# zju3dv/disprcnn

Measured on AMD Instinct MI355X. Metric: ROI cost-volumes/sec (112x112x48), higher is better.
Workload: dtype f32 (every convolution of the regressor, the three 32->1 heads included: split-f16 -- each fp32 value carried as hi + lo fp16, 3 f16-MFMA products per fp32 product, f32 accumulate; fp32-class error, tests/test_hip_s16.py.  Head gather and soft-argmin: f32 VALU); 1 GPU; Config A: per ROI pair, features [32,28,28]x2 -> concat cost volume [64,12,28,28] (folded into the first 3D layer's loads, never written) -> 3D stacked-hourglass regressor -> trilinear x4 + softmax + soft-argmin -> disparity [112,112]; maxdisp=48, mindisp=0, parallelism=roi-shard x1 (no collective), weights=closed-form synthetic (disprcnn_amd.utils.synth), BN stats calibrated fixture

## Files before the change

### disprcnn_amd/csrc/convs16.hip

```cpp
#include <hip/hip_runtime.h>
#include <stdint.h>

#include <type_traits>

#include "../../include/disprcnn_hip.h"
#include "s16_cvrows.h"
#include "s16_ovf.h"
#include "s16_tilemap.h"

typedef float f32x4 __attribute__((ext_vector_type(4)));
typedef float f32x16 __attribute__((ext_vector_type(16)));
typedef unsigned u32x4 __attribute__((ext_vector_type(4)));
typedef unsigned u32x2 __attribute__((ext_vector_type(2)));
typedef _Float16 f16x8 __attribute__((ext_vector_type(8)));
typedef _Float16 f16x4 __attribute__((ext_vector_type(4)));

#define GLOBAL_PTR(p) ((const __attribute__((address_space(1))) void*)(p))
#define LDS_PTR(p) ((__attribute__((address_space(3))) void*)(p))
#define S16_WAITCNT(vm, lgkm) (((vm) & 15) | (7 << 4) | ((lgkm) << 8) | (((vm) >> 4) << 14))

namespace {

constexpr int PV = 128;
constexpr int CPB = PV * 16;
constexpr int RING = 3;

template <int KW, bool CV, int RT = 1, int WT = 28, bool RES = false, bool Y32 = false, bool HEAD = false>
__global__ __launch_bounds__(256) __attribute__((amdgpu_waves_per_eu(1, 1))) void convs16_kernel(const drc_s16conv_params p) {
    static_assert(!HEAD || (KW == 2 && !CV && RT == 1 && !RES && !Y32), "the fused cout-1 head is a form of the 32 -> 32 full-resolution layer");
    static_assert(!CV || (KW == 4 && RT == 1 && WT == 28 && !RES && !Y32), "the cost-volume form: 64 virtual input channels, full-resolution rows, RS16 output");
    extern __shared__ __attribute__((aligned(16))) char lds[];
    if constexpr (CV) {
        s16cv::s16_cvrows_run<1>(p, lds);
        return;
    }
    constexpr int TX = WT;
    constexpr int SX = WT + 2;
    constexpr int RPW = 4 / KW;
    constexpr int CBI = KW / 2;
    constexpr int SROWS = RPW * RT + 2;
    static_assert(RT * WT <= 32, "tile shape");
    constexpr int SLAB = CBI * 8 * CPB;
    constexpr int NL = CBI * 8 * (PV / 64) / 4;
    constexpr int OWN = 16 / KW;
    constexpr int XW = 4096;
    constexpr int NR = RES ? 2 : 0;
    constexpr int NS = 2;
    static_assert(!(Y32 && (KW != 2 || RES)), "the blocked fp32 output exists for the 32-channel layers without residual");
    static_assert(RT == 1 ? SROWS * SX + 4 <= PV : (SROWS + 1) * SX + 4 <= PV, "slab plane too small (incl. the rows / columns the idle lanes over-read)");
    char* ring = lds;
    char* xchg = lds + RING * SLAB;
    char* pbuf = xchg + 2 * 4 * XW;

    const int wave = __builtin_amdgcn_readfirstlane(threadIdx.x >> 6);
    const int lane = threadIdx.x & 63;
    const int n_ = lane & 31, g = lane >> 5;
    const S16TileLane tln = s16_tile_lane<RT, WT>(n_, !(p.lo4 & 0x100));
    const int rl = tln.rl, xl = tln.xl;
    const int r = wave / KW, k = wave % KW;
    const int n_ct = p.cout / 32;
    const int ct = (int)((blockIdx.x >> 3) % n_ct);

    const int D = p.D, H = p.H, W = p.W;
    const int Wp = W + 2, Hp = H + 2;
    const long rowB = (long)Wp * 128;
    const long planeB = (long)Hp * rowB;
    const long xcbB = (long)(D + 2) * planeB;
    const long xnB = (long)CBI * xcbB;
    const int cbo = p.cout / 32;
    const long ynB = (long)cbo * xcbB;
    const long b_rowB = (long)Wp * 64, b_planeB = (long)Hp * b_rowB, b_cbB = (long)(D + 2) * b_planeB, b_nB = (long)(p.cout / 16) * b_cbB;

    f16x8 wh[27], wl[27];
    {
        const char* wb = (const char*)p.w + ((long)(ct * KW + k) * 54) * 1024 + lane * 16;
#pragma unroll
        for (int t = 0; t < 27; ++t) {
            wh[t] = *(const f16x8*)(wb + (t * 2) * 1024);
            wl[t] = *(const f16x8*)(wb + (t * 2 + 1) * 1024);
        }
    }
    float sc[OWN], sh[OWN];
#pragma unroll
    for (int e = 0; e < OWN; ++e) {
        const int reg = k * OWN + e;
        const int co = ct * 32 + (reg & 3) + 8 * (reg >> 2) + 4 * g;
        sc[e] = p.scale[co];
        sh[e] = p.shift[co];
    }
    f16x8 w1h = {}, w1l = {};
    if constexpr (HEAD) {
        const char* wb = (const char*)p.w1 + (long)k * 2048 + lane * 16;
        w1h = *(const f16x8*)wb;
        w1l = *(const f16x8*)(wb + 1024);
    }
    int srcrow[2], srcx[2];
    bool srcok[2];
#pragma unroll
    for (int h = 0; h < 2; ++h) {
        const int v = h * 64 + lane;
        srcok[h] = v < SROWS * SX;
        const int rr = srcok[h] ? v / SX : 0;
        srcrow[h] = rr;
        srcx[h] = srcok[h] ? v - rr * SX : 0;
    }
    const unsigned bfrag = (unsigned)(((k >> 1) * 8 + (k & 1) * 2 + g) * CPB + ((r * RT + rl) * SX + xl) * 16);
    const __attribute__((address_space(3))) char* ringl = (const __attribute__((address_space(3))) char*)ring;
    typedef const __attribute__((address_space(3))) f16x8 lds_frag;

    const int n_xt = (W + TX - 1) / TX, n_yt = (H + RPW * RT - 1) / (RPW * RT);
    const int Dw = (D + 2) / 3 * 3;
    const unsigned xcd = blockIdx.x & 7, qx = (blockIdx.x >> 3) / n_ct, per_xcd = (gridDim.x >> 3) / n_ct;
    const unsigned cols_unit = (unsigned)n_yt * n_xt;

    struct Col { unsigned n; int y0, x0; bool valid; };
    auto col_of = [&](unsigned it) __attribute__((always_inline)) {
        const unsigned j = it * per_xcd + qx;
        const unsigned nl = j / cols_unit;
        const unsigned rem = j - nl * cols_unit;
        const int yb = (int)(rem / n_xt), xt = (int)(rem - (unsigned)yb * n_xt);
        Col c;
        c.n = nl * 8 + xcd;
        c.valid = c.n < (unsigned)p.N;
        c.y0 = yb * RPW * RT;
        c.x0 = xt * TX;
        return c;
    };
    struct Src { const char* a; unsigned v0, v1; };
    auto src_of = [&](const Col& c) __attribute__((always_inline)) {
        Src q;
        q.a = (const char*)p.x + (long)c.n * xnB;
        q.v0 = (unsigned)((long)(c.y0 + srcrow[0]) * rowB + (long)(c.x0 + srcx[0]) * 16);
        q.v1 = (unsigned)((long)(c.y0 + srcrow[1]) * rowB + (long)(c.x0 + srcx[1]) * 16);
        return q;
    };
    auto stage = [&](const Src& q, int pl, int slot) __attribute__((always_inline)) {
        char* dst = ring + slot * SLAB;
        const __amdgpu_buffer_rsrc_t ra = __builtin_amdgcn_make_buffer_rsrc((void*)q.a, 0, 0x7FFFFF00, 0x00020000);
        const unsigned va[2] = {q.v0, q.v1};
#pragma unroll
        for (int i = 0; i < NL; ++i) {
            const int id = wave * NL + i;
            const int cb = id >> 4, c = (id >> 1) & 7, h = id & 1;
            const int so = (int)((long)cb * xcbB + (long)(pl + 1) * planeB + (long)c * (Wp * 16));
            __builtin_amdgcn_raw_ptr_buffer_load_lds(ra, LDS_PTR(dst + (cb * 8 + c) * CPB + h * 1024), 16, va[h], so, 0, 0);
        }
    };
    const long hs_planeB = (long)H * W * 48, hs_nB = (long)D * hs_planeB;
    struct Ctx { char* y16b; char* y32b; const char* resb; char* hsb; unsigned o16, o32, ohs; bool ok; };
    auto ctx_of = [&](const Col& c) __attribute__((always_inline)) {
        Ctx q;
        q.hsb = HEAD ? (char*)p.head + (long)c.n * hs_nB : (char*)p.w;
        q.ohs = (unsigned)(((long)(c.y0 + r * RT + rl) * W + (c.x0 + xl)) * 48 + g * 32);
        q.y16b = p.y16 ? (char*)p.y16 + (long)c.n * ynB : (char*)p.w;
        q.y32b = p.y32 ? (char*)p.y32 + (long)c.n * b_nB : (char*)p.w;
        q.resb = p.res ? (const char*)p.res + (long)c.n * ynB : (const char*)p.w;
        const int yl = c.y0 + r * RT + rl;
        q.ok = tln.ok && yl < H && c.x0 + xl < W;
        if constexpr (KW == 2) {
            q.o16 = (unsigned)((long)ct * xcbB + planeB + (long)(yl + 1) * rowB + (long)(k * 2 + g) * (Wp * 16) + (long)(c.x0 + xl + 1) * 16);
            q.o32 = (unsigned)((long)(2 * ct + k) * b_cbB + b_planeB + (long)(yl + 1) * b_rowB + (long)(c.x0 + xl + 1) * 64 + g * 16);
        } else {
            q.o16 = (unsigned)((long)ct * xcbB + planeB + (long)(yl + 1) * rowB + (long)((k >> 1) * 2 + g) * (Wp * 16) + (long)(c.x0 + xl + 1) * 16 + (k & 1) * 8);
            q.o32 = (unsigned)((long)(2 * ct + (k >> 1)) * b_cbB + b_planeB + (long)(yl + 1) * b_rowB + (long)(c.x0 + xl + 1) * 64 + (k & 1) * 32 + g * 16);
        }
        return q;
    };
    const unsigned lo_off = (unsigned)(4 * Wp * 16);
    const float relu_lo = p.relu ? 0.f : -65504.f;
    const unsigned n16 = p.y16 ? 0x7FFFFF00u : 0u, n32 = p.y32 ? 0x7FFFFF00u : 0u, nres = p.res ? 0x7FFFFF00u : 0u;

    Col ccur = col_of(0);
    if (!ccur.valid) return;
    S16Ovf og;
#pragma unroll
    for (int e = 0; e < OWN; ++e) { og.see_raw(sc[e], 3.0e38f); og.see_raw(sh[e], 3.0e38f); }
    Src s_cur = src_of(ccur), s_next = s_cur;
    Ctx cx_cur = ctx_of(ccur), cx_prev = cx_cur;
    cx_prev.ok = false;

    f32x16 acc[3];
    u32x4 resv[3][2];
#pragma unroll
    for (int a_ = 0; a_ < 3; ++a_)
#pragma unroll
        for (int e = 0; e < 16; ++e) acc[a_][e] = 0.f;
#pragma unroll
    for (int a_ = 0; a_ < 3; ++a_) resv[a_][0] = resv[a_][1] = (u32x4){0u, 0u, 0u, 0u};
    f32x16 pkeep = {};
    float SC[5] = {0.f, 0.f, 0.f, 0.f, 0.f}, SB[5] = {0.f, 0.f, 0.f, 0.f, 0.f};
    stage(s_cur, 0, 0);
    stage(s_cur, 1 < D ? 1 : D, 1);
    __builtin_amdgcn_s_waitcnt(S16_WAITCNT(NL, 15));
    unsigned gs = 0;

    auto step = [&](int t, auto JT, auto KT) __attribute__((always_inline)) {
        constexpr int J = decltype(JT)::value;
        constexpr int KIND = decltype(KT)::value;
        constexpr bool COMPUTE = KIND != 3;
        constexpr int A0 = (J + 1) % 3, A1 = J, A2 = (J + 2) % 3;
        asm volatile("" ::: "memory");
        __builtin_amdgcn_s_waitcnt(S16_WAITCNT(NL + NS + NR, 0));
        __builtin_amdgcn_s_barrier();
        asm volatile("" ::: "memory");
        const bool fcur = t >= 2, pcur = t >= 1;
        const int qf = fcur ? t - 2 : Dw - 2 + t, qp = pcur ? t - 1 : Dw - 1;
        const __amdgpu_buffer_rsrc_t resr = __builtin_amdgcn_make_buffer_rsrc((void*)(pcur ? cx_cur.resb : cx_prev.resb), 0, nres, 0x00020000);
        const unsigned p_o16 = pcur ? cx_cur.o16 : cx_prev.o16;
        const bool p_ok = (pcur ? cx_cur.ok : cx_prev.ok) && qp >= 0 && qp < D;
        if constexpr (RES) {
            const unsigned po = p_ok ? (unsigned)((long)qp * planeB) : 0x80000000u;
            if constexpr (KW == 2) {
                resv[J][0] = __builtin_amdgcn_raw_buffer_load_b128(resr, p_o16 + po, 0, 0);
                resv[J][1] = __builtin_amdgcn_raw_buffer_load_b128(resr, p_o16 + lo_off + po, 0, 0);
            } else {
                const u32x2 a_ = __builtin_amdgcn_raw_buffer_load_b64(resr, p_o16 + po, 0, 0);
                const u32x2 b_ = __builtin_amdgcn_raw_buffer_load_b64(resr, p_o16 + lo_off + po, 0, 0);
                resv[J][0] = (u32x4){a_.x, a_.y, 0u, 0u};
                resv[J][1] = (u32x4){b_.x, b_.y, 0u, 0u};
            }
        }
        {
            const int tp = t + 2;
            const bool nxt = tp >= Dw;
            Src q;
            q.a = nxt ? s_next.a : s_cur.a;
            q.v0 = nxt ? s_next.v0 : s_cur.v0;
            q.v1 = nxt ? s_next.v1 : s_cur.v1;
            int pl = nxt ? tp - Dw : tp;
            pl = pl < D ? pl : D;
            stage(q, pl, (J + 2) % 3);
        }
        const __amdgpu_buffer_rsrc_t y16r = __builtin_amdgcn_make_buffer_rsrc(fcur ? cx_cur.y16b : cx_prev.y16b, 0, n16, 0x00020000);
        const __amdgpu_buffer_rsrc_t y32r = __builtin_amdgcn_make_buffer_rsrc(fcur ? cx_cur.y32b : cx_prev.y32b, 0, n32, 0x00020000);
        const unsigned f_o16 = fcur ? cx_cur.o16 : cx_prev.o16, f_o32 = fcur ? cx_cur.o32 : cx_prev.o32;
        const bool f_ok = (fcur ? cx_cur.ok : cx_prev.ok) && qf >= 0 && qf < D;
        f32x4 part[4];
        {
            const char* xb = xchg + ((gs - 1) & 1) * (4 * XW) + (r * KW) * XW + lane * 16;
            if constexpr (KW == 2) {
                part[0] = *(const f32x4*)(xb + (k * 2) * 1024);
                part[1] = *(const f32x4*)(xb + XW + (k * 2) * 1024);
                part[2] = *(const f32x4*)(xb + (k * 2 + 1) * 1024);
                part[3] = *(const f32x4*)(xb + XW + (k * 2 + 1) * 1024);
            } else {
#pragma unroll
                for (int q = 0; q < 4; ++q) part[q] = *(const f32x4*)(xb + q * XW + k * 1024);
            }
        }
        f32x4 pin[4];
        if constexpr (HEAD) {
            const char* pb = pbuf + ((gs - 1) & 1) * (2 * XW) + r * XW + lane * 16;
#pragma unroll
            for (int q = 0; q < 4; ++q) pin[q] = *(const f32x4*)(pb + q * 1024);
        }
        if constexpr (RES) {
            __builtin_amdgcn_s_waitcnt(S16_WAITCNT(2 * NL + NS + NR, 15));
            __builtin_amdgcn_sched_barrier(0);
        }
        float v[OWN];
        _Float16 vh[OWN], vl[OWN];
        const unsigned long long og_keep = S16Ovf::lanes(f_ok);
        auto fin = [&](int e) __attribute__((always_inline)) {
            float s_;
            if constexpr (KW == 2) s_ = part[(e >> 2) * 2][e & 3] + part[(e >> 2) * 2 + 1][e & 3];
            else s_ = (part[0][e] + part[1][e]) + (part[2][e] + part[3][e]);
            float x_ = s_ * sc[e] + sh[e];
            if constexpr (RES) {
                const _Float16 rh = __builtin_bit_cast(f16x8, resv[(J + 2) % 3][0])[e], rl_ = __builtin_bit_cast(f16x8, resv[(J + 2) % 3][1])[e];
                x_ += (float)rh + (float)rl_;
            }
            x_ = __builtin_amdgcn_fmed3f(x_, relu_lo, 65504.f);
            og.see(x_, og_keep);
            v[e] = x_;
            vh[e] = (_Float16)x_;
            vl[e] = (_Float16)(x_ - (float)vh[e]);
        };
        auto stores = [&]() __attribute__((always_inline)) {
            if constexpr (Y32) {
                const unsigned po32 = f_ok ? (unsigned)((long)qf * b_planeB) : 0x80000000u;
                __builtin_amdgcn_raw_buffer_store_b128(__builtin_bit_cast(u32x4, (f32x4){v[0], v[1], v[2], v[3]}), y32r, f_o32 + po32, 0, 0);
                __builtin_amdgcn_raw_buffer_store_b128(__builtin_bit_cast(u32x4, (f32x4){v[4], v[5], v[6], v[7]}), y32r, f_o32 + 32 + po32, 0, 0);
            } else {
                const unsigned po = f_ok ? (unsigned)((long)qf * planeB) : 0x80000000u;
                if constexpr (KW == 2) {
                    f16x8 hi, lo;
#pragma unroll
                    for (int e = 0; e < 8; ++e) { hi[e] = vh[e]; lo[e] = vl[e]; }
                    __builtin_amdgcn_raw_buffer_store_b128(__builtin_bit_cast(u32x4, hi), y16r, f_o16 + po, 0, 0);
                    __builtin_amdgcn_raw_buffer_store_b128(__builtin_bit_cast(u32x4, lo), y16r, f_o16 + lo_off + po, 0, 0);
                } else {
                    f16x4 hi, lo;
#pragma unroll
                    for (int e = 0; e < 4; ++e) { hi[e] = vh[e]; lo[e] = vl[e]; }
                    __builtin_amdgcn_raw_buffer_store_b64(__builtin_bit_cast(u32x2, hi), y16r, f_o16 + po, 0, 0);
                    __builtin_amdgcn_raw_buffer_store_b64(__builtin_bit_cast(u32x2, lo), y16r, f_o16 + lo_off + po, 0, 0);
                }
            }
        };
        auto publish = [&]() __attribute__((always_inline)) {
            const f32x16 a = acc[A2];
            char* xb = xchg + (gs & 1) * (4 * XW) + wave * XW + lane * 16;
#pragma unroll
            for (int q = 0; q < 4; ++q) *(f32x4*)(xb + q * 1024) = (f32x4){a[q * 4], a[q * 4 + 1], a[q * 4 + 2], a[q * 4 + 3]};
#pragma unroll
            for (int e = 0; e < 16; ++e) acc[A2][e] = 0.f;
        };
        float o_[5];
        f32x16 z_ = {};
        f16x8 bh_ = {}, bl_ = {};
        auto head_update = [&](int jj) __attribute__((always_inline)) {
            if constexpr (HEAD) {
                const bool first = t == 3;
                const float p0 = pkeep[3 * jj] + pin[(3 * jj) >> 2][(3 * jj) & 3];
                const float p1 = pkeep[3 * jj + 1] + pin[(3 * jj + 1) >> 2][(3 * jj + 1) & 3];
                const float p2 = pkeep[3 * jj + 2] + pin[(3 * jj + 2) >> 2][(3 * jj + 2) & 3];
                o_[jj] = SC[jj] + (first ? 0.f : p2);
                SC[jj] = (first ? 0.f : SB[jj]) + p1;
                SB[jj] = p0;
            }
        };
        auto head_store = [&]() __attribute__((always_inline)) {
            if constexpr (HEAD) {
                const bool scur = t >= 4;
                const int ps = scur ? t - 4 : Dw - 4 + t;
                const bool ok_ = k == 0 && (scur ? cx_cur.ok : cx_prev.ok) && ps >= 0 && ps < D;
                const __amdgpu_buffer_rsrc_t hsr = __builtin_amdgcn_make_buffer_rsrc(scur ? cx_cur.hsb : cx_prev.hsb, 0, 0x7FFFFF00, 0x00020000);
                const unsigned oh_ = scur ? cx_cur.ohs : cx_prev.ohs;
                const unsigned po = ok_ ? (unsigned)((long)ps * hs_planeB) : 0x80000000u;
                __builtin_amdgcn_raw_buffer_store_b128(__builtin_bit_cast(u32x4, (f32x4){o_[0], o_[1], o_[2], o_[3]}), hsr, oh_ + po, 0, 0);
                __builtin_amdgcn_raw_buffer_store_b32(__builtin_bit_cast(unsigned, o_[4]), hsr, oh_ + 16 + (g ? 0x80000000u : po), 0, 0);
            }
        };
        auto head_mfma = [&](int i) __attribute__((always_inline)) {
            if constexpr (HEAD) {
                if (i == 0) {
#pragma unroll
                    for (int e = 0; e < 8; ++e) { bh_[e] = vh[e]; bl_[e] = vl[e]; }
                    z_ = __builtin_amdgcn_mfma_f32_32x32x16_f16(w1h, bh_, z_, 0, 0, 0);
                } else if (i == 1) {
                    z_ = __builtin_amdgcn_mfma_f32_32x32x16_f16(w1h, bl_, z_, 0, 0, 0);
                } else {
                    z_ = __builtin_amdgcn_mfma_f32_32x32x16_f16(w1l, bh_, z_, 0, 0, 0);
                    pkeep = z_;
                    if (k == 1) {
                        char* pb = pbuf + (gs & 1) * (2 * XW) + r * XW + lane * 16;
#pragma unroll
                        for (int q = 0; q < 4; ++q) *(f32x4*)(pb + q * 1024) = (f32x4){z_[q * 4], z_[q * 4 + 1], z_[q * 4 + 2], z_[q * 4 + 3]};
                    }
                }
            }
        };
        if constexpr (COMPUTE) {
            constexpr bool K0 = KIND != 2, K2 = KIND != 1;
            const __attribute__((address_space(3))) char* sb = ringl + J * SLAB + bfrag;
            f16x8 bh[2], bl[2];
            bh[0] = *(lds_frag*)(sb);
            bl[0] = *(lds_frag*)(sb + 4 * CPB);
#pragma unroll
            for (int q = 0; q < 9; ++q) {
                const int kh = q / 3, kw = q - kh * 3;
                if (q + 1 < 9) {
                    const int kh1 = (q + 1) / 3, kw1 = (q + 1) - kh1 * 3;
                    bh[(q + 1) & 1] = *(lds_frag*)(sb + (kh1 * SX + kw1) * 16);
                    bl[(q + 1) & 1] = *(lds_frag*)(sb + 4 * CPB + (kh1 * SX + kw1) * 16);
                }
                const f16x8 h_ = bh[q & 1], l_ = bl[q & 1];
                const int t0 = kh * 3 + kw, t1 = 9 + t0, t2 = 18 + t0;
                if (q == OWN && !HEAD) stores();
                if (q < 8) {
                    if (K0) acc[A0] = __builtin_amdgcn_mfma_f32_32x32x16_f16(wh[t0], h_, acc[A0], 0, 0, 0);
                    acc[A1] = __builtin_amdgcn_mfma_f32_32x32x16_f16(wh[t1], h_, acc[A1], 0, 0, 0);
                    if (K2) acc[A2] = __builtin_amdgcn_mfma_f32_32x32x16_f16(wh[t2], h_, acc[A2], 0, 0, 0);
                    if (K0) acc[A0] = __builtin_amdgcn_mfma_f32_32x32x16_f16(wh[t0], l_, acc[A0], 0, 0, 0);
                    acc[A1] = __builtin_amdgcn_mfma_f32_32x32x16_f16(wh[t1], l_, acc[A1], 0, 0, 0);
                    if (K2) acc[A2] = __builtin_amdgcn_mfma_f32_32x32x16_f16(wh[t2], l_, acc[A2], 0, 0, 0);
                    if (K0) acc[A0] = __builtin_amdgcn_mfma_f32_32x32x16_f16(wl[t0], h_, acc[A0], 0, 0, 0);
                    acc[A1] = __builtin_amdgcn_mfma_f32_32x32x16_f16(wl[t1], h_, acc[A1], 0, 0, 0);
                    if (K2) acc[A2] = __builtin_amdgcn_mfma_f32_32x32x16_f16(wl[t2], h_, acc[A2], 0, 0, 0);
                    if (q < OWN) fin(q);
                    if (q < 5) head_update(q);
                    if (q == 5) head_store();
                    __builtin_amdgcn_sched_barrier(0);
                } else {
                    if (K2) acc[A2] = __builtin_amdgcn_mfma_f32_32x32x16_f16(wh[t2], h_, acc[A2], 0, 0, 0);
                    if (K0) acc[A0] = __builtin_amdgcn_mfma_f32_32x32x16_f16(wh[t0], h_, acc[A0], 0, 0, 0);
                    head_mfma(0);
                    if (K2) acc[A2] = __builtin_amdgcn_mfma_f32_32x32x16_f16(wh[t2], l_, acc[A2], 0, 0, 0);
                    acc[A1] = __builtin_amdgcn_mfma_f32_32x32x16_f16(wh[t1], h_, acc[A1], 0, 0, 0);
                    if (K2) acc[A2] = __builtin_amdgcn_mfma_f32_32x32x16_f16(wl[t2], h_, acc[A2], 0, 0, 0);
                    __builtin_amdgcn_sched_barrier(0);
                    head_mfma(1);
                    if (K0) acc[A0] = __builtin_amdgcn_mfma_f32_32x32x16_f16(wh[t0], l_, acc[A0], 0, 0, 0);
                    acc[A1] = __builtin_amdgcn_mfma_f32_32x32x16_f16(wh[t1], l_, acc[A1], 0, 0, 0);
                    if (K0) acc[A0] = __builtin_amdgcn_mfma_f32_32x32x16_f16(wl[t0], h_, acc[A0], 0, 0, 0);
                    acc[A1] = __builtin_amdgcn_mfma_f32_32x32x16_f16(wl[t1], h_, acc[A1], 0, 0, 0);
                    publish();
                    head_mfma(2);
                }
            }
        } else {
#pragma unroll
            for (int e = 0; e < OWN; ++e) fin(e);
            if constexpr (HEAD) {
#pragma unroll
                for (int jj = 0; jj < 5; ++jj) head_update(jj);
                head_store();
                head_mfma(0); head_mfma(1); head_mfma(2);
            } else {
                stores();
            }
            publish();
        }
        ++gs;
    };
    using I0 = std::integral_constant<int, 0>;
    using I1 = std::integral_constant<int, 1>;
    using I2 = std::integral_constant<int, 2>;
    using I3 = std::integral_constant<int, 3>;
#pragma unroll 1
    for (unsigned it = 0;; ++it) {
        const Col cnext = col_of(it + 1);
        s_next = cnext.valid ? src_of(cnext) : s_cur;
        step(0, I0{}, I1{});
        step(1, I1{}, I0{});
        if (Dw == 3) {
            step(2, I2{}, I2{});
        } else {
            step(2, I2{}, I0{});
#pragma unroll 1
            for (int t0 = 3; t0 + 3 < Dw; t0 += 3) {
                step(t0, I0{}, I0{});
                step(t0 + 1, I1{}, I0{});
                step(t0 + 2, I2{}, I0{});
            }
            step(Dw - 3, I0{}, I0{});
            step(Dw - 2, I1{}, I0{});
            step(Dw - 1, I2{}, I2{});
        }
        if (!cnext.valid) break;
        cx_prev = cx_cur;
        cx_cur = ctx_of(cnext);
        s_cur = s_next;
    }
    step(Dw, I0{}, I3{});
    step(Dw + 1, I1{}, I3{});
    if constexpr (HEAD) {
        step(Dw + 2, I2{}, I3{});
        const bool ok_ = k == 0 && cx_cur.ok;
        const __amdgpu_buffer_rsrc_t hsr = __builtin_amdgcn_make_buffer_rsrc(cx_cur.hsb, 0, 0x7FFFFF00, 0x00020000);
        const unsigned po = ok_ ? (unsigned)((long)(D - 1) * hs_planeB) : 0x80000000u;
        __builtin_amdgcn_raw_buffer_store_b128(__builtin_bit_cast(u32x4, (f32x4){SC[0], SC[1], SC[2], SC[3]}), hsr, cx_cur.ohs + po, 0, 0);
        __builtin_amdgcn_raw_buffer_store_b32(__builtin_bit_cast(unsigned, SC[4]), hsr, cx_cur.ohs + 16 + (g ? 0x80000000u : po), 0, 0);
    }
    og.flush(p.ovf);
}

template <int KW, bool CV, int RT, int WT, bool RES, bool Y32, bool HEAD = false>
int launch2(const drc_s16conv_params& p, hipStream_t stream) {
    constexpr int CBI = KW / 2;
    constexpr int SLAB = CBI * 8 * CPB;
    constexpr int XW = 4096;
    constexpr size_t lds = CV ? (size_t)s16cv::LDS_BYTES : RING * SLAB + 2 * 4 * XW + (HEAD ? 2 * 2 * XW : 0);
    static_assert(lds <= 160 * 1024, "LDS");
    static bool attr_done = false;
    if (!attr_done) {
        (void)hipFuncSetAttribute((const void*)convs16_kernel<KW, CV, RT, WT, RES, Y32, HEAD>, hipFuncAttributeMaxDynamicSharedMemorySize, 160 * 1024);
        attr_done = true;
    }
    constexpr int rows = (4 / KW) * RT;
    const long columns = (long)p.N * ((p.H + rows - 1) / rows) * ((p.W + WT - 1) / WT);
    const int n_ct = p.cout / 32;
    long blocks = 256;
    while (blocks > 8 * n_ct && blocks / (2 * n_ct) >= columns) blocks /= 2;
    if constexpr (CV) blocks = s16cv::s16_cvrows_blocks<1>(p);
    hipLaunchKernelGGL((convs16_kernel<KW, CV, RT, WT, RES, Y32, HEAD>), dim3((unsigned)blocks), dim3(256), lds, stream, p);
    return (int)hipGetLastError();
}

template <int KW, bool CV, int RT = 1, int WT = 28>
int launch(const drc_s16conv_params& p, hipStream_t stream) {
    if (p.head) {
        if constexpr (KW == 2 && !CV && RT == 1) return launch2<KW, CV, RT, WT, false, false, true>(p, stream);
        else return -4;
    }
    if (p.y32) {
        if constexpr (KW == 2 && !CV && RT == 1) return launch2<KW, CV, RT, WT, false, true>(p, stream);
        else return -4;
    }
    if constexpr (CV) return launch2<KW, CV, RT, WT, false, false>(p, stream);
    else return p.res ? launch2<KW, CV, RT, WT, true, false>(p, stream) : launch2<KW, CV, RT, WT, false, false>(p, stream);
}

}

extern "C" int drc_conv3d_k3_s16_supported(int cin, int cout, int D, int H, int W) {
    if (cin != 32 && cin != 64) return 0;
    if (cout != 32 && cout != 64) return 0;
    return D > 0 && H > 0 && W > 0;
}

extern "C" int drc_conv3d_k3_s16_fwd(const drc_s16conv_params* pp, void* stream) {
    if (!pp) return -1;
    const drc_s16conv_params& p = *pp;
    const bool cv = p.left || p.right;
    if (!p.w || !p.scale || !p.shift) return -1;
    if (p.head) {
        if (!p.w1 || p.y16 || p.y32 || p.res || cv) return -1;
        if (p.cin != 32 || p.cout != 32 || p.W % 28 || p.D < 6 || p.D % 3) return -4;
        if ((long)p.D * p.H * p.W * 48 >= 0x7FFFFF00L) return -5;
    } else if (!p.y16 == !p.y32) return -1;
    if (p.y32 && (p.res || p.cin != 32 || p.W <= 14)) return -4;
    if (cv && p.res) return -4;
    if (cv ? (!p.left || !p.right || p.cin != 64) : !p.x) return -1;
    if (p.N < 0) return -2;
    if (!drc_conv3d_k3_s16_supported(p.cin, p.cout, p.D, p.H, p.W)) return -4;
    if (cv && p.W <= 14) return -4;
    if (p.N == 0) return 0;
    const long unit16 = (long)(p.cout / 32) * (p.D + 2) * (p.H + 2) * (p.W + 2) * 128;
    if (unit16 >= 0x7FFFFF00L / 2) return -5;
    hipStream_t s = (hipStream_t)stream;
    if (drc_conv3d_k3_s16_wide(pp)) return drc_conv3d_k3_s16_wide_fwd(pp, stream);
    if (cv) return launch<4, true>(p, s);
    if (p.W <= 7) return p.cin == 32 ? launch<2, false, 4, 7>(p, s) : launch<4, false, 4, 7>(p, s);
    if (p.W <= 14) return p.cin == 32 ? launch<2, false, 2, 14>(p, s) : launch<4, false, 2, 14>(p, s);
    return p.cin == 32 ? launch<2, false>(p, s) : launch<4, false>(p, s);
}
```

Baseline: 58490 ROI cost-volumes/s.

## Fold head depth-tap reduction into rotated 1x1 head MFMA weights

The fused 32->1 head conv previously computed all per-depth partial products and then combined the three depth taps with scalar shift registers (SC/SB) after the MFMA. Now three depth-rotated copies of the head weights are staged in LDS, and each step loads the copy that lines up with the current plane, so the MFMA accumulator itself sums across depth taps. Each step then reads out one slot and writes only five floats to the cross-wave exchange instead of sixteen. This removes per-step VALU shuffling and LDS exchange traffic. In return it adds LDS weight reloads, a masking pass at column boundaries, one extra drain step with a barrier, and a shift of the store pipeline by one plane.

```diff
diff --git a/disprcnn_amd/csrc/convs16.hip b/disprcnn_amd/csrc/convs16.hip
--- a/disprcnn_amd/csrc/convs16.hip
+++ b/disprcnn_amd/csrc/convs16.hip
@@ -51,6 +51,7 @@
     char* ring = lds;
     char* xchg = lds + RING * SLAB;
     char* pbuf = xchg + 2 * 4 * XW;
+    char* w1buf = pbuf + 2 * 2 * XW;
 
     const int wave = __builtin_amdgcn_readfirstlane(threadIdx.x >> 6);
     const int lane = threadIdx.x & 63;
@@ -88,11 +89,20 @@
         sc[e] = p.scale[co];
         sh[e] = p.shift[co];
     }
-    f16x8 w1h = {}, w1l = {};
+    unsigned w1_keep = ~0u;
     if constexpr (HEAD) {
-        const char* wb = (const char*)p.w1 + (long)k * 2048 + lane * 16;
-        w1h = *(const f16x8*)wb;
-        w1l = *(const f16x8*)(wb + 1024);
+        const int i_ = lane & 31, gp_ = (i_ >> 2) & 1, r_ = (i_ & 3) + 4 * (i_ >> 3);
+        w1_keep = r_ < 15 && r_ % 3 == 2 ? 0u : ~0u;
+#pragma unroll
+        for (int R = 0; R < 3; ++R) {
+            int rr = r_;
+            if (r_ < 15) rr = r_ / 3 * 3 + (R + 1 - r_ % 3 + 3) % 3;
+            const int src = (rr & 3) + 8 * (rr >> 2) + 4 * gp_ + (lane & 32);
+            const char* wb = (const char*)p.w1 + (long)k * 2048 + src * 16;
+            char* wd = w1buf + (wave * 3 + R) * 2048 + lane * 16;
+            *(f16x8*)wd = *(const f16x8*)wb;
+            *(f16x8*)(wd + 1024) = *(const f16x8*)(wb + 1024);
+        }
     }
     int srcrow[2], srcx[2];
     bool srcok[2];
@@ -187,16 +197,17 @@
         for (int e = 0; e < 16; ++e) acc[a_][e] = 0.f;
 #pragma unroll
     for (int a_ = 0; a_ < 3; ++a_) resv[a_][0] = resv[a_][1] = (u32x4){0u, 0u, 0u, 0u};
-    f32x16 pkeep = {};
-    float SC[5] = {0.f, 0.f, 0.f, 0.f, 0.f}, SB[5] = {0.f, 0.f, 0.f, 0.f, 0.f};
+    f32x16 Z = {};
+    float hk[5] = {0.f, 0.f, 0.f, 0.f, 0.f};
     stage(s_cur, 0, 0);
     stage(s_cur, 1 < D ? 1 : D, 1);
     __builtin_amdgcn_s_waitcnt(S16_WAITCNT(NL, 15));
     unsigned gs = 0;
 
-    auto step = [&](int t, auto JT, auto KT) __attribute__((always_inline)) {
+    auto step = [&](int t, auto JT, auto KT, auto HT) __attribute__((always_inline)) {
         constexpr int J = decltype(JT)::value;
         constexpr int KIND = decltype(KT)::value;
+        constexpr int HM = decltype(HT)::value;
         constexpr bool COMPUTE = KIND != 3;
         constexpr int A0 = (J + 1) % 3, A1 = J, A2 = (J + 2) % 3;
         asm volatile("" ::: "memory");
@@ -248,11 +259,12 @@
                 for (int q = 0; q < 4; ++q) part[q] = *(const f32x4*)(xb + q * XW + k * 1024);
             }
         }
-        f32x4 pin[4];
+        float hp_[5] = {0.f, 0.f, 0.f, 0.f, 0.f};
         if constexpr (HEAD) {
-            const char* pb = pbuf + ((gs - 1) & 1) * (2 * XW) + r * XW + lane * 16;
-#pragma unroll
-            for (int q = 0; q < 4; ++q) pin[q] = *(const f32x4*)(pb + q * 1024);
+            const char* pb = pbuf + ((gs - 1) & 1) * (2 * XW) + r * XW;
+            const f32x4 a_ = *(const f32x4*)(pb + lane * 16);
+            hp_[0] = a_[0]; hp_[1] = a_[1]; hp_[2] = a_[2]; hp_[3] = a_[3];
+            hp_[4] = *(const float*)(pb + 1024 + lane * 4);
         }
         if constexpr (RES) {
             __builtin_amdgcn_s_waitcnt(S16_WAITCNT(2 * NL + NS + NR, 15));
@@ -307,23 +319,45 @@
             for (int e = 0; e < 16; ++e) acc[A2][e] = 0.f;
         };
         float o_[5];
-        f32x16 z_ = {};
-        f16x8 bh_ = {}, bl_ = {};
-        auto head_update = [&](int jj) __attribute__((always_inline)) {
+        f16x8 bh_ = {}, bl_ = {}, ah_ = {}, al_ = {};
+        auto head_wload = [&]() __attribute__((always_inline)) {
+            if constexpr (HEAD && HM != 2) {
+                constexpr int R = (J + 1) % 3;
+                const char* wd = w1buf + (wave * 3 + R) * 2048 + lane * 16;
+                ah_ = *(const f16x8*)wd;
+                al_ = *(const f16x8*)(wd + 1024);
+                if constexpr (HM == 1) {
+                    unsigned m_ = w1_keep;
+                    asm volatile("" : "+v"(m_));
+                    const u32x4 mm = {m_, m_, m_, m_};
+                    ah_ = __builtin_bit_cast(f16x8, __builtin_bit_cast(u32x4, ah_) & mm);
+                    al_ = __builtin_bit_cast(f16x8, __builtin_bit_cast(u32x4, al_) & mm);
+                }
+            }
+        };
+        auto head_readout = [&]() __attribute__((always_inline)) {
             if constexpr (HEAD) {
-                const bool first = t == 3;
-                const float p0 = pkeep[3 * jj] + pin[(3 * jj) >> 2][(3 * jj) & 3];
-                const float p1 = pkeep[3 * jj + 1] + pin[(3 * jj + 1) >> 2][(3 * jj + 1) & 3];
-                const float p2 = pkeep[3 * jj + 2] + pin[(3 * jj + 2) >> 2][(3 * jj + 2) & 3];
-                o_[jj] = SC[jj] + (first ? 0.f : p2);
-                SC[jj] = (first ? 0.f : SB[jj]) + p1;
-                SB[jj] = p0;
+                constexpr int M = (J + 2) % 3;
+                float c_[5];
+#pragma unroll
+                for (int jj = 0; jj < 5; ++jj) { c_[jj] = Z[3 * jj + M]; Z[3 * jj + M] = 0.f; }
+                if constexpr (HM == 1) {
+#pragma unroll
+                    for (int jj = 0; jj < 5; ++jj) Z[3 * jj + (J + 1) % 3] = 0.f;
+                }
+                if (k == 1) {
+                    char* pb = pbuf + (gs & 1) * (2 * XW) + r * XW;
+                    *(f32x4*)(pb + lane * 16) = (f32x4){c_[0], c_[1], c_[2], c_[3]};
+                    *(float*)(pb + 1024 + lane * 4) = c_[4];
+                }
+#pragma unroll
+                for (int jj = 0; jj < 5; ++jj) { o_[jj] = hk[jj] + hp_[jj]; hk[jj] = c_[jj]; }
             }
         };
         auto head_store = [&]() __attribute__((always_inline)) {
             if constexpr (HEAD) {
-                const bool scur = t >= 4;
-                const int ps = scur ? t - 4 : Dw - 4 + t;
+                const bool scur = t >= 5;
+                const int ps = scur ? t - 5 : Dw - 5 + t;
                 const bool ok_ = k == 0 && (scur ? cx_cur.ok : cx_prev.ok) && ps >= 0 && ps < D;
                 const __amdgpu_buffer_rsrc_t hsr = __builtin_amdgcn_make_buffer_rsrc(scur ? cx_cur.hsb : cx_prev.hsb, 0, 0x7FFFFF00, 0x00020000);
                 const unsigned oh_ = scur ? cx_cur.ohs : cx_prev.ohs;
@@ -333,21 +367,15 @@
             }
         };
         auto head_mfma = [&](int i) __attribute__((always_inline)) {
-            if constexpr (HEAD) {
+            if constexpr (HEAD && HM != 2) {
                 if (i == 0) {
 #pragma unroll
                     for (int e = 0; e < 8; ++e) { bh_[e] = vh[e]; bl_[e] = vl[e]; }
-                    z_ = __builtin_amdgcn_mfma_f32_32x32x16_f16(w1h, bh_, z_, 0, 0, 0);
+                    Z = __builtin_amdgcn_mfma_f32_32x32x16_f16(ah_, bh_, Z, 0, 0, 0);
                 } else if (i == 1) {
-                    z_ = __builtin_amdgcn_mfma_f32_32x32x16_f16(w1h, bl_, z_, 0, 0, 0);
+                    Z = __builtin_amdgcn_mfma_f32_32x32x16_f16(ah_, bl_, Z, 0, 0, 0);
                 } else {
-                    z_ = __builtin_amdgcn_mfma_f32_32x32x16_f16(w1l, bh_, z_, 0, 0, 0);
-                    pkeep = z_;
-                    if (k == 1) {
-                        char* pb = pbuf + (gs & 1) * (2 * XW) + r * XW + lane * 16;
-#pragma unroll
-                        for (int q = 0; q < 4; ++q) *(f32x4*)(pb + q * 1024) = (f32x4){z_[q * 4], z_[q * 4 + 1], z_[q * 4 + 2], z_[q * 4 + 3]};
-                    }
+                    Z = __builtin_amdgcn_mfma_f32_32x32x16_f16(al_, bh_, Z, 0, 0, 0);
                 }
             }
         };
@@ -379,8 +407,9 @@
                     acc[A1] = __builtin_amdgcn_mfma_f32_32x32x16_f16(wl[t1], h_, acc[A1], 0, 0, 0);
                     if (K2) acc[A2] = __builtin_amdgcn_mfma_f32_32x32x16_f16(wl[t2], h_, acc[A2], 0, 0, 0);
                     if (q < OWN) fin(q);
-                    if (q < 5) head_update(q);
-                    if (q == 5) head_store();
+                    if (q == 0) head_readout();
+                    if (q == 1) head_store();
+                    if (q == 6) head_wload();
                     __builtin_amdgcn_sched_barrier(0);
                 } else {
                     if (K2) acc[A2] = __builtin_amdgcn_mfma_f32_32x32x16_f16(wh[t2], h_, acc[A2], 0, 0, 0);
@@ -403,9 +432,9 @@
 #pragma unroll
             for (int e = 0; e < OWN; ++e) fin(e);
             if constexpr (HEAD) {
-#pragma unroll
-                for (int jj = 0; jj < 5; ++jj) head_update(jj);
+                head_readout();
                 head_store();
+                head_wload();
                 head_mfma(0); head_mfma(1); head_mfma(2);
             } else {
                 stores();
@@ -418,40 +447,51 @@
     using I1 = std::integral_constant<int, 1>;
     using I2 = std::integral_constant<int, 2>;
     using I3 = std::integral_constant<int, 3>;
+    using H0 = std::integral_constant<int, 0>;
+    using H1 = std::integral_constant<int, HEAD ? 1 : 0>;
+    using H2 = std::integral_constant<int, HEAD ? 2 : 0>;
 #pragma unroll 1
     for (unsigned it = 0;; ++it) {
         const Col cnext = col_of(it + 1);
         s_next = cnext.valid ? src_of(cnext) : s_cur;
-        step(0, I0{}, I1{});
-        step(1, I1{}, I0{});
+        step(0, I0{}, I1{}, H0{});
+        step(1, I1{}, I0{}, H0{});
         if (Dw == 3) {
-            step(2, I2{}, I2{});
+            step(2, I2{}, I2{}, H1{});
         } else {
-            step(2, I2{}, I0{});
+            step(2, I2{}, I0{}, H1{});
 #pragma unroll 1
             for (int t0 = 3; t0 + 3 < Dw; t0 += 3) {
-                step(t0, I0{}, I0{});
-                step(t0 + 1, I1{}, I0{});
-                step(t0 + 2, I2{}, I0{});
-            }
-            step(Dw - 3, I0{}, I0{});
-            step(Dw - 2, I1{}, I0{});
-            step(Dw - 1, I2{}, I2{});
+                step(t0, I0{}, I0{}, H0{});
+                step(t0 + 1, I1{}, I0{}, H0{});
+                step(t0 + 2, I2{}, I0{}, H0{});
+            }
+            step(Dw - 3, I0{}, I0{}, H0{});
+            step(Dw - 2, I1{}, I0{}, H0{});
+            step(Dw - 1, I2{}, I2{}, H0{});
         }
         if (!cnext.valid) break;
         cx_prev = cx_cur;
         cx_cur = ctx_of(cnext);
         s_cur = s_next;
     }
-    step(Dw, I0{}, I3{});
-    step(Dw + 1, I1{}, I3{});
+    step(Dw, I0{}, I3{}, H0{});
+    step(Dw + 1, I1{}, I3{}, H0{});
     if constexpr (HEAD) {
-        step(Dw + 2, I2{}, I3{});
+        step(Dw + 2, I2{}, I3{}, H2{});
+        step(Dw + 3, I0{}, I3{}, H2{});
+        asm volatile("" ::: "memory");
+        __builtin_amdgcn_s_waitcnt(S16_WAITCNT(63, 0));
+        __builtin_amdgcn_s_barrier();
+        asm volatile("" ::: "memory");
+        const char* pb = pbuf + ((gs - 1) & 1) * (2 * XW) + r * XW;
+        const f32x4 a_ = *(const f32x4*)(pb + lane * 16);
+        const float b_ = *(const float*)(pb + 1024 + lane * 4);
         const bool ok_ = k == 0 && cx_cur.ok;
         const __amdgpu_buffer_rsrc_t hsr = __builtin_amdgcn_make_buffer_rsrc(cx_cur.hsb, 0, 0x7FFFFF00, 0x00020000);
         const unsigned po = ok_ ? (unsigned)((long)(D - 1) * hs_planeB) : 0x80000000u;
-        __builtin_amdgcn_raw_buffer_store_b128(__builtin_bit_cast(u32x4, (f32x4){SC[0], SC[1], SC[2], SC[3]}), hsr, cx_cur.ohs + po, 0, 0);
-        __builtin_amdgcn_raw_buffer_store_b32(__builtin_bit_cast(unsigned, SC[4]), hsr, cx_cur.ohs + 16 + (g ? 0x80000000u : po), 0, 0);
+        __builtin_amdgcn_raw_buffer_store_b128(__builtin_bit_cast(u32x4, (f32x4){hk[0] + a_[0], hk[1] + a_[1], hk[2] + a_[2], hk[3] + a_[3]}), hsr, cx_cur.ohs + po, 0, 0);
+        __builtin_amdgcn_raw_buffer_store_b32(__builtin_bit_cast(unsigned, hk[4] + b_), hsr, cx_cur.ohs + 16 + (g ? 0x80000000u : po), 0, 0);
     }
     og.flush(p.ovf);
 }
@@ -461,7 +501,7 @@
     constexpr int CBI = KW / 2;
     constexpr int SLAB = CBI * 8 * CPB;
     constexpr int XW = 4096;
-    constexpr size_t lds = CV ? (size_t)s16cv::LDS_BYTES : RING * SLAB + 2 * 4 * XW + (HEAD ? 2 * 2 * XW : 0);
+    constexpr size_t lds = CV ? (size_t)s16cv::LDS_BYTES : RING * SLAB + 2 * 4 * XW + (HEAD ? 2 * 2 * XW + 4 * 3 * 2048 : 0);
     static_assert(lds <= 160 * 1024, "LDS");
     static bool attr_done = false;
     if (!attr_done) {
```

Result: no change. 58990 ROI cost-volumes/s (median of 6 runs) (+0.9%).
